# alshai/rowbowt

Measured on AMD Instinct MI355X. Metric: reads/s (100 bp, count+locate), higher is better.
Workload: dtype u32/u64

## Files before the change

rowbowt_amd/csrc/k_runs.hip:

```cpp
#include <type_traits>

#include "rbg_runs2_device.hpp"
#include "rbg_chain_walk.hpp"
#include "rbg_locate_docs.hpp"
#include "rbg_jump.h"
#include "rbg_launch.hpp"

namespace rbg {
namespace {

struct PackedBits {
    const uint4 *__restrict__ cp;
    uint4 w;
    uint32_t widx, navail;
    uint64_t sr;
    __device__ __forceinline__ uint32_t next_word() {
        if (widx == 4) { w = *cp++; widx = 0; }
        const uint32_t v = w.x;
        w.x = w.y; w.y = w.z; w.z = w.w;
        ++widx;
        return v;
    }
    __device__ __forceinline__ uint32_t take(uint32_t nb) {
        if (navail < nb) { sr |= static_cast<uint64_t>(next_word()) << navail; navail += 32; }
        const uint32_t v = static_cast<uint32_t>(sr & ((uint64_t(1) << nb) - 1));
        sr >>= nb;
        navail -= nb;
        return v;
    }
};

template <bool GLDS>
__device__ __forceinline__ bool jump_probe_wave(const void *__restrict__ tab, const uint64_t nb, const bool probing, const JumpKey &key, uint32_t v[3],
                                                uint32_t &buckets, lds_byte *tile) {
    uint32_t state = probing ? kJumpNext : kJumpAbsent;
    uint64_t b = probing ? jump_home(jump_hash(key), nb) : 0u;
    uint64_t left = nb;
    while (__ballot(state == kJumpNext)) {
        const bool undecided = state == kJumpNext;
        uint32_t w[16];
        quad_fetch_issue<GLDS>(reinterpret_cast<uint64_t>(tab) + (undecided ? b : 0u) * kJumpBucketBytes, w, tile);
        quad_fetch_take<GLDS>(w, tile);
        if (undecided) {
            ++buckets;
            state = jump_bucket(w, key, v);
            b = jump_next(b, nb);
            if (--left == 0 && state == kJumpNext) state = kJumpAbsent;
        }
    }
    return state <= kJumpHit1;
}

__device__ __forceinline__ uint64_t uniform_u64(const uint64_t v) {
    const uint32_t lo = static_cast<uint32_t>(__builtin_amdgcn_readfirstlane(static_cast<uint32_t>(v)));
    const uint32_t hi = static_cast<uint32_t>(__builtin_amdgcn_readfirstlane(static_cast<uint32_t>(v >> 32)));
    return static_cast<uint64_t>(lo) | (static_cast<uint64_t>(hi) << 32);
}

struct StagedWords {
    const lds_u32 *codes;
    __device__ __forceinline__ uint32_t operator()(const uint32_t j) const { return codes[64u * j]; }
};

template <typename P, bool TOEHOLD, bool PACKED = false, bool STATS = false, bool GLDS = false, bool STAGE = false>
__global__ __launch_bounds__(512, STATS ? 2 : 4) void k_find_range_runs(const DevIndex ix, const void *__restrict__ src_a,
                                                        const void *__restrict__ src_b, const uint64_t N,
                                                        uint64_t *__restrict__ lo_out, uint64_t *__restrict__ hi_out,
                                                        uint64_t *__restrict__ ss_out, unsigned long long *__restrict__ stats,
                                                        const uint32_t *__restrict__ sel, const uint32_t *__restrict__ nsel) {
    const uint64_t Neff = sel ? static_cast<uint64_t>(*nsel) : N;
    const uint8_t *__restrict__ seqs = static_cast<const uint8_t *>(src_a);
    const uint64_t *__restrict__ off = static_cast<const uint64_t *>(src_b);
    const uint4 *__restrict__ chunks = static_cast<const uint4 *>(src_a);
    const uint2 *__restrict__ meta = static_cast<const uint2 *>(src_b);
    __shared__ uint8_t s_lut[256];
    __shared__ uint8_t s_lut2[256];
    __shared__ uint8_t s_mslot[4];
    __shared__ __align__(16) unsigned char s_tile[GLDS ? 8 * kTileBytes : 16];
    __shared__ uint32_t s_codes[STAGE ? 8 * kStageWords * 64 : 1];
    __shared__ uint64_t s_jump[STAGE ? 4 : 1];
    __shared__ uint32_t s_jump_k[STAGE ? 2 : 1];
    for (int t = threadIdx.x; t < 256; t += blockDim.x) {
        s_lut[t] = ix.lut[t];
        s_lut2[t] = ix.nmajor ? ix.lut2[t] : 0xFFu;
    }
    if (STAGE && threadIdx.x < 2) {
        const uint32_t t = threadIdx.x;
        s_jump[2 * t] = reinterpret_cast<uint64_t>(ix.jump) + (t ? ix.jump_buckets * kJumpBucketBytes : 0u);
        s_jump[2 * t + 1] = t ? ix.jump2_buckets : ix.jump_buckets;
        s_jump_k[t] = t ? ix.jump2_k : ix.jump_k;
    }
    RBG_RUN_SEARCH2_SHARED;
    const RunSearch2<P> S2 = stage_run_search2<P>(ix, s_tab_first, s_ent2, s_dir2, s_rec2, s_dyn);
    const uint32_t *tab_first = s_tab_first;
    lds_byte *tile = (lds_byte *)s_tile + (GLDS ? (threadIdx.x >> 6) * kTileBytes : 0u);
    if (PACKED || STAGE) {
        for (int t = threadIdx.x; t < 256; t += blockDim.x)
            if (s_lut2[t] != 0xFFu) s_mslot[s_lut2[t] & 3u] = s_lut[t];
        __syncthreads();
    }
    const uint32_t D = ix.run_ksteps, DMASK = ix.run_depth_mask | 1u;
    const uint32_t M = ix.nmajor;
    const uint32_t lane = threadIdx.x & (kWave - 1);
    lds_u32 *codes = (lds_u32 *)s_codes + (STAGE ? (threadIdx.x >> 6) * (kStageWords * 64u) + lane : 0u);
    const StageTab stage_tab{ix.stage_code[0], ix.stage_code[1], ix.stage_byte[0], ix.stage_byte[1], ix.stage_shift};
    const bool stage_on = STAGE && ix.stage_ok != 0 && M == 4;

    unsigned long long c_occ = 0, c_reads = 0;
    uint32_t c_matched = 0;
    unsigned long long st[kStatSearchN] = {0, 0, 0, 0, 0, 0, 0, 0};
    const uint64_t stride = static_cast<uint64_t>(gridDim.x) * blockDim.x;
    const uint64_t wave_first = static_cast<uint64_t>(blockIdx.x) * blockDim.x + (threadIdx.x & ~(kWave - 1));
    for (uint64_t base = wave_first; base < Neff; base += stride) {
        bool valid = base + lane < Neff;
        const uint64_t i = (sel && valid) ? static_cast<uint64_t>(sel[base + lane]) : base + lane;
        uint64_t beg = 0, p = 0;
        PackedBits bs{chunks, make_uint4(0, 0, 0, 0), 4u, 0u, 0ull};
        if (PACKED) {
            if (valid) {
                const uint2 mt = meta[i];
                if (mt.y & 0x80000000u) valid = false;
                else { p = mt.y; bs.cp = chunks + mt.x; }
            }
        } else if (valid) { beg = off[i]; p = off[i + 1]; }
        bool staged = false;
        if constexpr (STAGE && !PACKED) {
            if (stage_on && __ballot(valid && p - beg > kStageCap) == 0) {
                uint32_t nch = 0;
                const bool bad = valid && stage_read(reinterpret_cast<const uint4 *>(seqs), beg, p, stage_tab, codes, nch);
                if (STATS) st[kStChunks] += nch;
                staged = __ballot(bad) == 0;
                if (staged) { p -= beg; beg = 0; }
                else if (STATS) st[kStChunks] -= nch;
            }
        }
        auto walk = [&](auto staged_tag) __attribute__((always_inline)) {
            constexpr bool STAGED = decltype(staged_tag)::value;
            const uint64_t p_end = p;
            uint64_t p_min = p;
            const uint32_t m32 = static_cast<uint32_t>(p);
            uint64_t lo = 0, hi = ix.n - 1;
            uint64_t k = TOEHOLD ? ix.last_run_sample : 0;
            bool alive = valid;
            bool pend = false;
            uint32_t pend_d = 0, pend_rec = 0;
            uint64_t pend_e = 0;
            ByteCursor rd{reinterpret_cast<const uint4 *>(seqs), ~uint64_t(0), make_uint4(0, 0, 0, 0)};
            bool jumped = false;
            if constexpr (STAGED && sizeof(P) == 4) {
                if (ix.jump) {
                    const uint32_t nlev = ix.jump2_k ? 2u : 1u;
                    bool hit = valid;
                    uint32_t from = 0;
#pragma unroll 1
                    for (uint32_t lev = 0; lev < nlev; ++lev) {
                        const uint32_t K = __builtin_amdgcn_readfirstlane(s_jump_k[lev]);
                        const uint64_t tab = uniform_u64(s_jump[2 * lev]), nb = uniform_u64(s_jump[2 * lev + 1]);
                        const bool probing = hit && static_cast<uint32_t>(p) >= K;
                        JumpKey key = jump_key_from_codes(StagedWords{codes}, from, K);
                        if (lev) key.w[3] = static_cast<uint32_t>(lo);
                        from = K;
                        uint32_t v[3] = {0, 0, 0}, nbk = 0;
                        hit = jump_probe_wave<GLDS>(reinterpret_cast<const void *>(tab), nb, probing, key, v, nbk, tile);
                        if (hit) {
                            lo = v[0]; hi = v[1];
                            if (TOEHOLD) k = v[2] == 0xFFFFFFFFu ? ~uint64_t(0) : static_cast<uint64_t>(v[2]);
                            p -= K;
                            jumped = true;
                            if (STATS) st[kStSymbols] += K;
                        }
                        if (STATS) st[kStFtab] += nbk;
                        if constexpr (!STATS) {
                            if (probing && !hit && jump_absent_ends(ix.jump_complete, lev)) { alive = false; p = beg; }
                        }
                    }
                }
            }
            if (!jumped && valid && ix.ftab_k && p - beg >= ix.ftab_k) {
                uint64_t idx = 0;
                bool all_major = true;
                PackedBits probe = bs;
                if constexpr (STAGED) {
                    const uint32_t w0 = codes[0];
                    idx = ix.ftab_k >= 16u ? w0 : (w0 & ((1u << (2u * ix.ftab_k)) - 1u));
                } else if (PACKED) {
                    idx = probe.take(2 * ix.ftab_k);
                } else {
                    uint64_t pw = 1;
                    for (uint32_t t = 1; t <= ix.ftab_k; ++t) {
                        const uint32_t mm = s_lut2[rd.at(p - t)];
                        all_major = all_major && mm != 0xFFu;
                        idx += (mm & 3u) * pw;
                        pw *= M;
                    }
                }
                uint64_t flo, fhi2, fk;
                if (STATS) { if (!STAGED) p_min = p - ix.ftab_k; if (all_major) st[kStFtab] += 1; }
                if (all_major && ftab_lookup<P>(ix, idx, flo, fhi2, fk)) {
// ... 79 lines not shown
                    if (STATS) st[kStSymbols] += adv;
                    const uint64_t c_inside = r.c_upto - r.c_before;
                    if (c_inside == 0) {
                        alive = false;
                    } else {
                        if (TOEHOLD) {
                            if (r.inside) k = k - adv;
                            else { pend = true; pend_d = d; pend_rec = rec; pend_e = r.samp_e; k = 0; }
                        }
                        lo = r.F + r.c_before;
                        hi = lo + c_inside - 1;
                        p = p_next;
                    }
                }
            }
            if (TOEHOLD && alive && pend) {
                k += run_step_sample2<P>(ix, S2, pend_d, pend_rec, pend_e);
                if (STATS) st[kStResample] += 1;
            }
            if (STATS && !PACKED && !STAGED && p_end > p_min) st[kStChunks] += ((p_end - 1) >> 4) - (p_min >> 4) + 1;
            if (STATS && PACKED && valid) st[kStChunks] += (p_end + 63) >> 6;
            if (!alive) { lo = 1; hi = 0; k = 0; }
            if (valid) {
                lo_out[i] = lo;
                hi_out[i] = hi;
                if (TOEHOLD) ss_out[i] = k;
                c_reads += 1;
                if (alive) { c_matched += 1; c_occ += hi - lo + 1; }
            }
        };
        if (STAGE && staged) walk(std::integral_constant<bool, STAGE>{}); else walk(std::false_type{});
    }
    c_reads = wave_sum(c_reads);
    const unsigned long long w_matched = wave_sum(static_cast<unsigned long long>(c_matched));
    c_occ = wave_sum(c_occ);
    if (lane == 0 && c_reads) {
        atomicAdd(&ix.counters[0], c_reads);
        if (w_matched) atomicAdd(&ix.counters[1], w_matched);
        if (c_occ) atomicAdd(&ix.counters[2], c_occ);
    }
    if (STATS) {
#pragma unroll
        for (int t = 0; t < kStatSearchN; ++t) {
            const unsigned long long v = wave_sum(st[t]);
            if (lane == 0 && v) atomicAdd(&stats[t], v);
        }
    }
}

template <typename P> struct ChunkR { static constexpr int v = 8; };

template <typename P, typename OUT = uint64_t, bool STATS = false, bool SUB = false, bool HI8 = false>
__global__ __launch_bounds__(256, 4) void k_locate_fill_runs2(const DevIndex ix, const uint64_t *__restrict__ lo,
                                                          const uint64_t *__restrict__ hi, const uint64_t *__restrict__ k,
                                                          const uint64_t N, const uint64_t max_hits,
                                                          const uint64_t *__restrict__ loc_off, OUT *__restrict__ locs,
                                                          const uint64_t *__restrict__ sub, const uint32_t *__restrict__ order,
                                                          const uint64_t *__restrict__ skeys, unsigned long long *__restrict__ stats) {
    constexpr int kChunkR = ChunkR<P>::v;
    using Stage = ChainStage<P, kChunkR, SUB, true, HI8>;
    __shared__ Stage S;
    chain_fill_walk<P, OUT, STATS, SUB, HI8, kChunkR, 1>(ix, S, lo, hi, k, N, max_hits, loc_off, locs, sub, order, skeys, stats,
                                                         [&](const uint64_t k1, unsigned long long &cost) { return run_phi<P, STATS>(ix, k1, cost); });
}

extern __shared__ unsigned long long locate_docs_lds[];
template <typename P, bool LOCS>
__global__ __launch_bounds__(kLocDocBlock) void k_locate_docs_runs2(const DevIndex ix, const DocTable t, const uint64_t *__restrict__ lo,
                                                                   const uint64_t *__restrict__ hi, const uint64_t *__restrict__ k, const uint64_t N,
                                                                   const uint64_t max_hits, const uint32_t *__restrict__ order,
                                                                   const uint64_t *__restrict__ skeys, uint64_t *__restrict__ sets,
                                                                   uint32_t *__restrict__ ndocs_out, uint32_t *__restrict__ nodoc_out,
                                                                   unsigned long long *__restrict__ doc_reads, unsigned long long *__restrict__ doc_locs) {
    locate_docs_walk<P, LOCS>(ix, t, locate_docs_lds, lo, hi, k, N, max_hits, order, skeys, sets, ndocs_out, nodoc_out, doc_reads, doc_locs,
                              [&](const uint64_t k1, unsigned long long &cost) { return run_phi<P>(ix, k1, cost); });
}

}

int launch_find_range_runs_impl(const DevIndex &ix, const LaunchCfg &cfg, const void *src_a, const void *src_b, uint64_t N,
                                uint64_t *lo, uint64_t *hi, uint64_t *ssamp, void *stream, bool packed, unsigned long long *stats,
                                const uint32_t *sel = nullptr, const uint32_t *nsel = nullptr) {
    if (N == 0) return 0;
    const size_t lds = run_search2_lds(ix);
    static const bool glds = [] { const char *e = std::getenv("RBG_REC_FETCH"); return !(e && std::strcmp(e, "quad") == 0); }();
    static const bool stage = [] { const char *e = std::getenv("RBG_STAGE_READS"); return !(e && e[0] == '0'); }();
    if (stats && packed) return static_cast<int>(hipErrorNotSupported);
    const LaunchCfg c = runs512_cfg(cfg);
    const dim3 grid(sel ? std::min(grid_for(c, N), 256) : grid_for(c, N)), block(512);
    return with_pos(ix.pos_bytes, [&](auto p) { return with_flag(ssamp != nullptr, [&](auto toe) {
        auto search = [&](auto pk, auto sts, auto gl, auto sg) {
            constexpr bool GL = decltype(gl)::value, SG = decltype(sg)::value;
            return launch_lds(k_find_range_runs<pos_t<decltype(p)>, decltype(toe)::value, decltype(pk)::value, decltype(sts)::value, GL, SG>, grid, block, lds,
                              (GL ? 8 * kTileBytes : 0) + (SG ? 8 * kStageWaveBytes : 0), stream, ix, src_a, src_b, N, lo, hi, ssamp, stats, sel, nsel);
        };
        auto fetch = [&](auto pk, auto sts) {
            if constexpr (!decltype(pk)::value) { if (glds && stage && !sel) return search(no, sts, yes, yes); }
            return glds ? search(pk, sts, yes, no) : search(pk, sts, no, no);
        };
        if (stats) return fetch(no, yes);
        return packed ? fetch(yes, no) : fetch(no, no);
    }); });
}

int launch_find_range_runs(const DevIndex &ix, const LaunchCfg &cfg, const uint8_t *seqs, const uint64_t *off, uint64_t N,
                           uint64_t *lo, uint64_t *hi, uint64_t *ssamp, void *stream, unsigned long long *stats) {
    return launch_find_range_runs_impl(ix, cfg, seqs, off, N, lo, hi, ssamp, stream, false, stats);
}

int launch_find_range_runs_sel(const DevIndex &ix, const LaunchCfg &cfg, const uint8_t *seqs, const uint64_t *off, uint64_t N, uint64_t *lo,
                               uint64_t *hi, uint64_t *ssamp, const uint32_t *sel, const uint32_t *nsel, void *stream) {
    return launch_find_range_runs_impl(ix, cfg, seqs, off, N, lo, hi, ssamp, stream, false, nullptr, sel, nsel);
}

int launch_find_range_runs_packed(const DevIndex &ix, const LaunchCfg &cfg, const uint2 *meta, const uint4 *chunks, uint64_t N,
                                  uint64_t *lo, uint64_t *hi, uint64_t *ssamp, void *stream) {
    return launch_find_range_runs_impl(ix, cfg, chunks, meta, N, lo, hi, ssamp, stream, true, nullptr);
}

int launch_locate_fill_runs(const DevIndex &ix, const LaunchCfg &cfg, const uint64_t *lo, const uint64_t *hi, const uint64_t *k,
                            uint64_t N, uint64_t max_hits, const uint64_t *loc_off, uint64_t *locs, const uint64_t *sub,
                            const void *order, const uint64_t *skeys, void *stream, unsigned long long *stats, uint32_t *locs32) {
    if (N == 0) return 0;
    const dim3 grid(grid_for(cfg, N)), block(256);
    const uint32_t *perm = static_cast<const uint32_t *>(order);
    return chain_fill_variants(ix, stats, sub, locs, locs32, [&](auto p, auto sts, auto sb, auto h8, auto *dst) {
        return launch_grid(k_locate_fill_runs2<pos_t<decltype(p)>, std::remove_pointer_t<decltype(dst)>, decltype(sts)::value, decltype(sb)::value, decltype(h8)::value>,
                           grid, block, 0, stream, ix, lo, hi, k, N, max_hits, loc_off, dst, sub, perm, skeys, stats);
    });
}

int launch_locate_doc_hits_runs(const DevIndex &ix, const DocTable &t, const uint64_t *lo, const uint64_t *hi, const uint64_t *k, uint64_t N, uint64_t max_hits,
                                const void *order, const uint64_t *skeys, uint64_t *sets, uint32_t *ndocs_out, uint32_t *nodoc_out, uint64_t *doc_reads,
                                uint64_t *doc_locs, void *stream) {
    if (t.ndocs == 0 || t.ndocs > kLocDocLdsDocs) return static_cast<int>(hipErrorInvalidValue);
    if (N == 0) return 0;
    const dim3 grid(locate_docs_grid(N)), block(kLocDocBlock);
    const uint32_t *perm = static_cast<const uint32_t *>(order);
    unsigned long long *dr = reinterpret_cast<unsigned long long *>(doc_reads), *dl = reinterpret_cast<unsigned long long *>(doc_locs);
    const size_t lds = locate_docs_lds_bytes(t.ndocs, t.ndir, doc_locs != nullptr);
    return with_pos(ix.pos_bytes, [&](auto p) { return with_flag(doc_locs != nullptr, [&](auto lc) {
        return launch_lds(k_locate_docs_runs2<pos_t<decltype(p)>, decltype(lc)::value>, grid, block, lds, 0, stream,
                          ix, t, lo, hi, k, N, max_hits, perm, skeys, sets, ndocs_out, nodoc_out, dr, dl);
    }); });
}

}
```

rowbowt_amd/csrc/rbg_dev.h:

```cpp
#pragma once

#include <hip/hip_runtime.h>

#include <algorithm>
#include <cstddef>
#include <cstdint>
#include <cstdio>
#include <vector>

#include "rbg_mkdir.hpp"
#include "rbg_fl.hpp"
#include "rbg_isa.hpp"

namespace rbg {

template <typename P>
struct RunEnt {
    P start;
    P cum;
};

template <typename P>
struct PhiEnt {
    P pos;
// ... 61 lines not shown
    uint32_t nruns;
};

constexpr int kLdsSyms = 8;
constexpr int kMaxMajor = 4;

struct DevRunTab2 {
    uint64_t F;
    uint64_t first;
    uint64_t dir_off;
    uint32_t dir_shift, pad;
};
static_assert(sizeof(DevRunTab2) == 32, "two 16-byte reads per record");
constexpr uint32_t kRunHotShiftBit = 56;
struct RunDir64 { uint32_t count, hi; };
constexpr uint32_t kRec2Pivots = 12;
constexpr uint32_t kRec2Overflow = 16u;
constexpr uint32_t kRec2Compact = 32u;
constexpr uint32_t kRec2CompactIn = 10;
struct alignas(64) RunRec2 {
    uint32_t e0;
    uint32_t hi;
    uint32_t meta;
    uint32_t cum_end;
    uint32_t ent[kRec2Pivots];
};
static_assert(sizeof(RunRec2) == 64, "one sector per bucket");
constexpr uint32_t kRunFillShift = 30;
struct PhiEnt12 { uint32_t pos_lo, base_lo, base_hi; };
static_assert(sizeof(PhiEnt12) == 12, "three words per entry");
constexpr uint32_t kPhiSuperShift = 16;

constexpr int kMaxRunDepth = 8;
constexpr int kLdsRunDepth = 5;
constexpr int kMaxLdsRunTabs = kLdsSyms + 16 + 64 + 256 + 1024 + kLdsRunDepth;


struct DevIndex {
    uint64_t n, r;
    uint64_t last_run_sample;
    const DevSym *syms;
    uint32_t sigma;
    uint32_t pos_bytes;
    const void *phi_ent;
    const void *phi_slots;
    const uint32_t *phi_ord;
    uint32_t phi_shift;
    uint32_t has_tsa;
    const uint64_t *mk_start, *mk_end, *mk_off, *mk_vals;
    uint64_t mk_nruns;
    const uint32_t *mk_bucket;
    uint32_t mk_shift;
    const MkRec *mk_rec;
    unsigned long long *counters;
    const uint8_t *lut;
    const DevSym *pairs;
    const DevSym *triples;
    const DevSym *quads;
    const DevSym *quints;
    const uint8_t *lut2;
    uint32_t nmajor;
    uint32_t kmer_steps;
    const void *ftab;
    uint32_t ftab_k;
    uint32_t phi_packed;
    const uint8_t *dense;
    uint32_t layout;
    uint32_t run_ksteps;
    uint32_t run_ntabs;
    const void *run_samp[kMaxRunDepth];
    uint32_t run_tab_first[kMaxRunDepth + 1];
    const uint32_t *phi_dir;
    uint32_t phi_dir_shift;
    uint32_t run_depth_mask;
    uint32_t phi_super_shift;
    uint32_t run_fill_shift;
    const void *run_ent2[kMaxRunDepth];
    const void *run_dir2[kMaxRunDepth];
    const DevRunTab2 *run_tabs2;
    const uint64_t *run_hot;
    uint32_t run_uni_depth;
    uint32_t run_uni_stride;
    uint32_t run_uni_shift;
    const RunRec2 *run_rec2[kMaxRunDepth];
    const uint64_t *phi_super;
    uint64_t phi_m;
    uint64_t phi_last_pos, phi_last_base;
    const uint64_t *order_docs;
    uint32_t order_ndocs, order_dbits, order_lowbits, order_obits;
    uint32_t stage_ok, stage_shift;
    uint32_t stage_code[2];
    uint32_t stage_byte[2];
    const void *jump;
    uint64_t jump_buckets;
    uint32_t jump_k;
    uint32_t jump2_k;
    uint64_t jump2_buckets;
    uint32_t jump_complete;
    uint32_t tmk_shift;
    const uint64_t *tmk_start, *tmk_end, *tmk_off, *tmk_vals;
    uint64_t tmk_nruns;
    const uint32_t *tmk_bucket;
    const MkRec *tmk_rec;
};

enum SearchStat {
    kStSteps = 0,
    kStSlots,
    kStDense,
    kStSearch,
    kStFtab,
    kStResample,
    kStChunks,
    kStSymbols,
    kStatSearchN
};
static_assert(kMkStatRuns == kStatSearchN + 2, "marker_span_arrays counts the run starts / ends it reads behind the search counters");
enum LocateStat {
    kLsPhiSteps = 0,
    kLsPhiOvf,
    kLsChains,
    kLsLocs,
    kStatLocateN
};

template <typename P>
struct SeedLogRec {
    P lo, hi;
    uint32_t qs, qe, mb, me;
};
struct SeedLogWin {
    uint32_t src, cnt;
};
struct SeedLog {
    unsigned char *base;
    uint64_t stride;
    uint32_t qs, qw;
    uint32_t *nsel;
    unsigned long long *stats = nullptr;
};
enum SeedStat {
    kSdMarkerQueries = kStatSearchN,
    kSdMarkerDir,
    kSdMarkerProbes,
    kSdMarkerOff,
    kSdMarkerVals,
    kSdSeedRecs,
    kSdSequences,
    kSeedStatN
};
constexpr uint32_t kSeedLogOverflow = 0xFFFFFFFFu;
constexpr uint32_t kSeedLogWindows = 6, kSeedLogSeedsDefault = 12;
inline size_t seed_log_rec_bytes(uint32_t pos_bytes) { return pos_bytes == 4 ? sizeof(SeedLogRec<uint32_t>) : sizeof(SeedLogRec<uint64_t>); }
inline size_t seed_log_stride(uint32_t pos_bytes, uint32_t seeds_per_read) {
    return 8 + static_cast<size_t>(seeds_per_read) * seed_log_rec_bytes(pos_bytes) + kSeedLogWindows * sizeof(SeedLogWin);
}
inline size_t seed_log_bytes(uint64_t N, uint32_t pos_bytes, uint32_t seeds_per_read) {
    return static_cast<size_t>(N) * seed_log_stride(pos_bytes, seeds_per_read) + 64 + (N + 4) * 4;
}
inline SeedLog make_seed_log(void *scratch, size_t bytes, uint64_t N, uint32_t pos_bytes) {
    SeedLog lg{nullptr, 0, 0, kSeedLogWindows, nullptr, nullptr};
    if (!scratch || N == 0 || (reinterpret_cast<uintptr_t>(scratch) & 15)) return lg;
    const size_t tail = 64 + (N + 4) * 4, fixed = 8 + kSeedLogWindows * sizeof(SeedLogWin), rec = seed_log_rec_bytes(pos_bytes);
    if (bytes < tail + N * (fixed + 2 * rec)) return lg;
    size_t q = ((bytes - tail) / N - fixed) / rec;
    if (q > 255) q = 255;
    lg.qs = static_cast<uint32_t>(q);
    lg.stride = fixed + q * rec;
    lg.base = static_cast<unsigned char *>(scratch);
    lg.nsel = reinterpret_cast<uint32_t *>(lg.base + ((N * lg.stride + 15) & ~size_t(15)));
    return lg;
}

struct ComposeTable {
    const void *ent;
    const void *samp;
    uint64_t nruns, total, F;
};
struct ComposedLevel {
    void *ent = nullptr;
    void *samp = nullptr;
    uint64_t entries = 0;
    std::vector<uint64_t> nruns, total, F, first;
};
int compose_levels_device(uint32_t pos_bytes, uint64_t n, uint32_t M, const ComposeTable *major, const void *g_start, const uint32_t *g_id,
                          const void *g_samp, uint64_t g_n, uint32_t kmax, bool with_samples, std::vector<ComposedLevel> &out, void *stream,
                          uint32_t keep_mask = 0 ,
                          bool *inputs_released = nullptr );

inline double host_memory_available() {
    double avail = 1e18;
    if (FILE *f = std::fopen("/proc/meminfo", "r")) {
        char line[256];
        while (std::fgets(line, sizeof line, f)) {
            unsigned long long kb = 0;
            if (std::sscanf(line, "MemAvailable: %llu kB", &kb) == 1) { avail = static_cast<double>(kb) * 1024.0; break; }
        }
        std::fclose(f);
    }
    unsigned long long mx = 0, cur = 0;
    bool have_mx = false, have_cur = false;
    if (FILE *f = std::fopen("/sys/fs/cgroup/memory.max", "r")) { have_mx = std::fscanf(f, "%llu", &mx) == 1; std::fclose(f); }
    if (FILE *f = std::fopen("/sys/fs/cgroup/memory.current", "r")) { have_cur = std::fscanf(f, "%llu", &cur) == 1; std::fclose(f); }
    if (have_mx && have_cur && mx > cur) avail = std::min(avail, static_cast<double>(mx - cur));
    else if (have_mx && have_cur) avail = 0;
    return avail;
}


struct LaunchCfg {
    int block_threads = 256;
    int max_blocks = 0;
};

int launch_find_range(const DevIndex &ix, const LaunchCfg &cfg, const uint8_t *seqs, const uint64_t *off, uint64_t N,
                      uint64_t *lo, uint64_t *hi, uint64_t *ssamp , void *stream);
int launch_find_range_runs(const DevIndex &ix, const LaunchCfg &cfg, const uint8_t *seqs, const uint64_t *off, uint64_t N,
                           uint64_t *lo, uint64_t *hi, uint64_t *ssamp , void *stream,
                           unsigned long long *stats = nullptr );
int launch_find_range_runs_sel(const DevIndex &ix, const LaunchCfg &cfg, const uint8_t *seqs, const uint64_t *off, uint64_t N, uint64_t *lo,
                               uint64_t *hi, uint64_t *ssamp , const uint32_t *sel, const uint32_t *nsel, void *stream);
int launch_find_range_runs_packed(const DevIndex &ix, const LaunchCfg &cfg, const uint2 *meta, const uint4 *chunks, uint64_t N,
                                  uint64_t *lo, uint64_t *hi, uint64_t *ssamp , void *stream);
int launch_locate_fill_runs(const DevIndex &ix, const LaunchCfg &cfg, const uint64_t *lo, const uint64_t *hi, const uint64_t *k,
                            uint64_t N, uint64_t max_hits, const uint64_t *loc_off, uint64_t *locs, const uint64_t *sub,
                            const void *order, const uint64_t *skeys, void *stream, unsigned long long *stats = nullptr ,
                            uint32_t *locs32 = nullptr);
int launch_lf_runs(const DevIndex &ix, const LaunchCfg &cfg, const uint64_t *lo, const uint64_t *hi, const uint8_t *sym, uint64_t N,
                   uint64_t *lo_out, uint64_t *hi_out, void *stream);
int launch_find_range_markers_runs(const DevIndex &ix, const LaunchCfg &cfg, const uint8_t *seqs, const uint64_t *off, uint64_t N,
                                   uint64_t wsize, uint64_t max_range, uint64_t *lo, uint64_t *hi, uint64_t *cnt, const uint64_t *mk_off,
                                   uint64_t *mk, bool fill, void *stream);
int launch_greedy_seed_runs(const DevIndex &ix, const LaunchCfg &cfg, const uint8_t *seqs, const uint64_t *off, uint64_t N,
                            uint64_t min_length, uint64_t *lo, uint64_t *hi, uint64_t *qs, uint64_t *qe, uint64_t *ss, void *stream,
                            unsigned long long *stats = nullptr );
int launch_marker_seeds_runs(const DevIndex &ix, const LaunchCfg &cfg, const uint8_t *seqs, const uint64_t *off, uint64_t N, uint64_t wsize,
                             uint64_t max_range, uint64_t *seed_cnt, uint64_t *mk_cnt, const uint64_t *seed_off, const uint64_t *mk_off,
                             uint64_t *seeds, uint64_t *mk, bool fill, void *stream, const SeedLog &lg, uint64_t ftab_k = 0 );
int launch_marker_lmems_runs(const DevIndex &ix, const LaunchCfg &cfg, const uint8_t *seqs, const uint64_t *off, uint64_t N, uint64_t total,
                             uint64_t wsize, uint64_t max_range, uint64_t ftab_k, uint64_t *rec_off, uint64_t *seeds, uint64_t *mk, bool fill,
                             void *stream);
int launch_greedy_seeds_list_runs(const DevIndex &ix, const LaunchCfg &cfg, const uint8_t *seqs, const uint64_t *off, uint64_t N, uint64_t min_length,
                                  bool w_sample, uint64_t *seed_cnt, const uint64_t *seed_off, uint64_t *lo, uint64_t *hi, uint64_t *qs, uint64_t *qe,
                                  uint64_t *ss , bool fill, void *stream);
int launch_toehold_chkpnts_runs(const DevIndex &ix, const LaunchCfg &cfg, const uint8_t *seqs, const uint64_t *off, uint64_t N, uint64_t wsize,
                                const uint64_t *slot_off, uint64_t *cnt, uint64_t *lo, uint64_t *hi, uint64_t *qs, uint64_t *qe, uint64_t *ss,
                                void *stream);
int launch_find_range_stats(const DevIndex &ix, const LaunchCfg &cfg, const uint8_t *seqs, const uint64_t *off, uint64_t N,
                            uint64_t *lo, uint64_t *hi, uint64_t *ssamp , unsigned long long *stats ,
                            void *stream);
size_t scan_tmp_bytes(uint64_t N);
int launch_locate_plan(const DevIndex &ix, const LaunchCfg &cfg, const uint64_t *lo, const uint64_t *hi, uint64_t N,
                       uint64_t max_hits, uint64_t *loc_off, void *tmp, size_t tmp_bytes, void *stream);
int launch_locate_fill(const DevIndex &ix, const LaunchCfg &cfg, const uint64_t *lo, const uint64_t *hi,
                       const uint64_t *k, uint64_t N, uint64_t max_hits, const uint64_t *loc_off, uint64_t *locs,
                       const uint64_t *sub ,
                       const void *order , void *stream,
                       unsigned long long *stats = nullptr ,
                       uint32_t *locs32 = nullptr );
size_t locate_order_ws_bytes(uint64_t N);
int launch_locate_order(const DevIndex &ix, const LaunchCfg &cfg, const uint64_t *k, uint64_t N, void *ws, size_t ws_bytes,
                        void *stream);
int launch_build_rank_slots(uint32_t pos_bytes, const void *ent, uint64_t nruns, uint64_t n, uint32_t shift, void *slots,
                            uint32_t *ord, unsigned long long *overflow, unsigned long long *dense_cursor, void *stream);
int launch_fill_dense(uint32_t pos_bytes, const void *ent, uint64_t n, uint32_t shift, const void *slots, const uint32_t *ord,
                      uint8_t *dense, void *stream);
size_t text_ws_bytes(uint64_t E);
int launch_copy16(const void *pinned_src, void *dst, uint64_t bytes, void *stream);
int launch_text_plan(const uint64_t *lo, const uint64_t *hi, const uint64_t *loc_off, const uint64_t *locs, uint64_t N, uint64_t E, const char *names,
                     const uint32_t *name_off, const uint64_t *doc_start, const char *doc_names, const uint32_t *doc_name_off, uint64_t ndocs,
                     uint64_t text_size, bool with_locs, const uint64_t *mk_off, const uint64_t *mk, void *ws, size_t ws_bytes, unsigned int *d_bad, void *stream);
void text_total_ptrs(void *ws, uint64_t E, const uint64_t **last_at, const uint32_t **last_len);
int launch_text_fill(const uint64_t *lo, const uint64_t *hi, const uint64_t *loc_off, const uint64_t *locs, uint64_t N, uint64_t E, const char *names,
                     const uint32_t *name_off, const uint64_t *doc_start, const char *doc_names, const uint32_t *doc_name_off, uint64_t ndocs,
                     uint64_t text_size, bool with_locs, const uint64_t *mk_off, const uint64_t *mk, void *ws, uint64_t total, char *text, void *stream);
struct SamBatch {
    uint64_t N, E;
    const uint64_t *lo, *hi, *a, *b;
    const uint8_t *rev;
    const uint64_t *line_off, *loc_off, *locs;
    const char *seqs, *quals;
    const uint64_t *roff;
    const char *names;
    const uint32_t *name_off;
    const uint64_t *doc_start;
    const char *doc_names;
    const uint32_t *doc_name_off;
    uint64_t ndocs, text_size;
};
int launch_sam_strands(const uint8_t *seqs, const uint64_t *off, uint64_t N, uint64_t total, uint8_t *out, uint64_t *off2, uint32_t cap, void *stream);
size_t sam_pick_tmp_bytes(uint64_t N);
int launch_sam_pick(const uint64_t *lo2, const uint64_t *hi2, const uint64_t *qs2, const uint64_t *qe2, const uint64_t *ss2, uint64_t N, uint64_t max_hits,
                    uint64_t *lo, uint64_t *hi, uint64_t *k, uint64_t *a, uint64_t *b, uint8_t *rev, uint64_t *nlines, uint64_t *line_off,
                    unsigned long long *counters, void *tmp, size_t tmp_bytes, uint32_t cap, void *stream);
size_t sam_ws_bytes(uint64_t E);
int launch_sam_plan(const SamBatch &B, void *ws, size_t ws_bytes, unsigned int *d_bad, uint32_t cap, void *stream);
void sam_total_ptrs(void *ws, uint64_t E, const uint64_t **last_at, const uint64_t **last_len);
int launch_sam_fill(const SamBatch &B, void *ws, uint64_t total, char *text, uint32_t cap, void *stream);
int launch_sam_offsets(void *ws, uint64_t E, void *stream);
int launch_extend_left(const DevIndex &ix, const uint8_t *seqs, const uint64_t *off, uint64_t N, const uint32_t *item_seq, const uint32_t *item_a,
                       const uint64_t *item_row, const uint64_t *item_limit, uint64_t M, uint32_t max_mismatch, void *out, unsigned int *d_err, uint32_t cap,
                       void *stream);
// ... 160 lines not shown
```

rowbowt_amd/csrc/rbg_jump.h:

```cpp
#pragma once

#include <cstdint>

#if defined(__HIPCC__)
#define RBG_JUMP_HD __host__ __device__ __forceinline__
#else
#define RBG_JUMP_HD inline
#endif

namespace rbg {

constexpr uint32_t kJumpMaxK = 64;
constexpr uint32_t kJumpMinK = 16;
constexpr uint32_t kJumpSlotWords = 8;
constexpr uint32_t kJumpBucketBytes = 64;
constexpr uint32_t kJumpEmptyTag = 0, kJumpFullTag = 1;
constexpr uint32_t kJumpDefaultK = 60;
constexpr uint64_t kJumpAutoMinBytes = uint64_t(256) << 20;

struct JumpKey {
    uint32_t w[4];
};

RBG_JUMP_HD void jump_key_mask(JumpKey &key, uint32_t K) {
// ... 9 lines not shown
}

RBG_JUMP_HD uint64_t jump_hash(const JumpKey &key) {
    const uint64_t a = key.w[0] | (static_cast<uint64_t>(key.w[1]) << 32);
    const uint64_t b = key.w[2] | (static_cast<uint64_t>(key.w[3]) << 32);
    uint64_t h = (a * 0x9E3779B97F4A7C15ull) ^ ((b + 0x632BE59BD9B4E019ull) * 0xC2B2AE3D27D4EB4Full);
    h ^= h >> 29;
    h *= 0xBF58476D1CE4E5B9ull;
    h ^= h >> 32;
    return h;
}

RBG_JUMP_HD uint64_t jump_home(uint64_t h, uint64_t nb) {
    return ((h >> 32) * nb) >> 32;
}

constexpr uint32_t kJumpHit0 = 0, kJumpHit1 = 1, kJumpAbsent = 2, kJumpNext = 3;
RBG_JUMP_HD uint32_t jump_bucket(const uint32_t w[16], const JumpKey &key, uint32_t v[3]) {
    for (uint32_t s = 0; s < 2; ++s) {
        const uint32_t *sl = w + kJumpSlotWords * s;
        if (sl[7] == kJumpEmptyTag) return kJumpAbsent;
        if (sl[0] == key.w[0] && sl[1] == key.w[1] && sl[2] == key.w[2] && sl[3] == key.w[3]) {
            v[0] = sl[4]; v[1] = sl[5]; v[2] = sl[6];
            return s;
        }
    }
    return kJumpNext;
}

RBG_JUMP_HD uint64_t jump_next(uint64_t b, uint64_t nb) { return b + 1 == nb ? 0 : b + 1; }

template <typename Load>
RBG_JUMP_HD bool jump_probe(const Load &load, uint64_t nb, const JumpKey &key, uint32_t v[3], uint32_t &buckets) {
    uint64_t b = jump_home(jump_hash(key), nb);
    for (uint64_t step = 0; step < nb; ++step) {
        ++buckets;
        uint32_t w[16];
        load(b, 0, w, w + 4);
        load(b, 1, w + 8, w + 12);
        const uint32_t r = jump_bucket(w, key, v);
        if (r != kJumpNext) return r != kJumpAbsent;
        b = jump_next(b, nb);
    }
    return false;
}

constexpr uint32_t kJump2MaxK = 48;
constexpr uint32_t kJump2MinK = 16;
constexpr uint32_t kJump2DefaultK = 40;

RBG_JUMP_HD JumpKey jump2_key(uint32_t s0, uint32_t s1, uint32_t s2, uint32_t K2, uint32_t parent_lo) {
    JumpKey key{{s0, s1, s2, 0u}};
    jump_key_mask(key, K2);
    key.w[3] = parent_lo;
    return key;
}

template <typename Word>
RBG_JUMP_HD JumpKey jump_key_from_codes(const Word &word, uint32_t from, uint32_t K) {
    const uint32_t w0 = from >> 4, sh = 2u * (from & 15u);
    const uint32_t c0 = word(w0), c1 = word(w0 + 1), c2 = word(w0 + 2), c3 = word(w0 + 3), c4 = word(w0 + 4);
    const auto funnel = [sh](uint32_t lo, uint32_t hi) { return static_cast<uint32_t>(((static_cast<uint64_t>(hi) << 32) | lo) >> sh); };
    JumpKey key{{funnel(c0, c1), funnel(c1, c2), funnel(c2, c3), funnel(c3, c4)}};
    jump_key_mask(key, K);
    return key;
}

template <typename Word>
RBG_JUMP_HD JumpKey jump2_key_from_codes(const Word &word, uint32_t K1, uint32_t K2, uint32_t parent_lo) {
    JumpKey key = jump_key_from_codes(word, K1, K2);
    key.w[3] = parent_lo;
    return key;
}

RBG_JUMP_HD JumpKey jump2_key_from_text(const uint8_t *codes, uint32_t K2, uint32_t parent_lo) {
    JumpKey key{{0, 0, 0, 0}};
    for (uint32_t t = 0; t < K2; ++t) jump_key_set(key, t, codes[K2 - 1 - t]);
    key.w[3] = parent_lo;
    return key;
}

inline uint64_t jump_buckets_for(uint64_t keys) { return keys ? keys : 1; }

constexpr uint32_t kJumpComplete1 = 1u, kJumpComplete2 = 2u;
struct JumpBuilt {
    bool stands;
    uint64_t words, inserted;
};
RBG_JUMP_HD bool jump_level_complete(const JumpBuilt &b) { return b.stands && b.words != 0 && b.inserted == b.words; }
RBG_JUMP_HD uint32_t jump_complete_mask(const JumpBuilt &l1, const JumpBuilt &l2, bool absent_ends) {
    if (!absent_ends || !l1.stands) return 0u;
    return (jump_level_complete(l1) ? kJumpComplete1 : 0u) | (jump_level_complete(l2) ? kJumpComplete2 : 0u);
}
RBG_JUMP_HD bool jump_absent_ends(uint32_t mask, uint32_t lev) { return ((mask >> lev) & 1u) != 0; }

}
```

Before: 2.417 billion.

## Add lean two-level jump-table kernel for exact-length reads, defer rest to runs search

Adds a small, high-occupancy kernel that handles reads whose length equals K1+K2. It stages each read into LDS, probes the two complete jump hash tables, and writes the range directly. Reads it cannot take are marked with a sentinel. The full runs search kernel then runs in a marked-only mode that skips already-resolved reads, using a reduced persistent grid. This trades one extra launch and an extra pass over lo_out for avoiding the heavy backward-search kernel on most 100 bp reads.

New measurement: 2.370 billion. -1.9%, worse.

```diff
diff --git a/rowbowt_amd/csrc/jump_lean.hip b/rowbowt_amd/csrc/jump_lean.hip
--- /dev/null
+++ b/rowbowt_amd/csrc/jump_lean.hip
@@ -0,0 +1,97 @@
+#include "rbg_jump_probe.hpp"
+#include "rbg_launch.hpp"
+
+namespace rbg {
+namespace {
+
+constexpr int kLeanBlock = 256;
+constexpr uint32_t kLeanWords = 8u;
+static_assert((kJumpMaxK + kJump2MaxK + 15u) / 16u <= kLeanWords, "a read the lean kernel takes fits its column");
+
+struct LeanColumn {
+    const lds_u32 *codes;
+    __device__ __forceinline__ uint32_t operator()(const uint32_t j) const { return codes[64u * j]; }
+};
+
+struct LeanIndex {
+    const void *tab1, *tab2;
+    uint64_t nb1, nb2;
+    uint32_t K1, K2;
+    StageTab stage;
+    unsigned long long *counters;
+};
+
+template <bool TOEHOLD>
+__global__ __launch_bounds__(kLeanBlock, 8) void k_jump_lean(const LeanIndex ix, const uint8_t *__restrict__ seqs, const uint64_t *__restrict__ off,
+                                                             const uint64_t N, uint64_t *__restrict__ lo_out, uint64_t *__restrict__ hi_out,
+                                                             uint64_t *__restrict__ ss_out) {
+    __shared__ uint32_t s_codes[(kLeanBlock / kWave) * kLeanWords * 64];
+    const uint32_t lane = threadIdx.x & (kWave - 1);
+    lds_u32 *codes = (lds_u32 *)s_codes + (threadIdx.x >> 6) * (kLeanWords * 64u) + lane;
+    const uint32_t K1 = ix.K1, K2 = ix.K2;
+    unsigned long long c_occ = 0;
+    uint32_t c_reads = 0, c_matched = 0;
+    const uint64_t stride = static_cast<uint64_t>(gridDim.x) * blockDim.x;
+    const uint64_t wave_first = static_cast<uint64_t>(blockIdx.x) * blockDim.x + (threadIdx.x & ~(kWave - 1));
+    for (uint64_t base = wave_first; base < N; base += stride) {
+        const uint64_t i = base + lane;
+        const bool valid = i < N;
+        uint64_t beg = 0, end = 0;
+        if (valid) { beg = off[i]; end = off[i + 1]; }
+        bool take = valid && jump_lean_takes(end - beg, K1, K2);
+        uint64_t lo = 1, hi = 0, k = 0;
+        bool hit = false;
+        if (__ballot(take)) {
+            uint32_t nch = 0;
+            const bool bad = stage_read(reinterpret_cast<const uint4 *>(seqs), take ? beg : 0u, take ? end : 0u, ix.stage, codes, nch);
+            take = take && !bad;
+            const JumpWordsClamped<LeanColumn> words{LeanColumn{codes}, kLeanWords};
+            uint32_t v[3] = {0, 0, 0}, nbk = 0;
+            const JumpKey key1 = jump_key_from_codes(words, 0u, K1);
+            hit = jump_probe_wave<false>(ix.tab1, ix.nb1, take, key1, v, nbk, nullptr);
+            const JumpKey key2 = jump2_key_from_codes(words, K1, K2, v[0]);
+            hit = jump_probe_wave<false>(ix.tab2, ix.nb2, hit, key2, v, nbk, nullptr);
+            if (hit) {
+                lo = v[0]; hi = v[1];
+                if (TOEHOLD) k = v[2] == 0xFFFFFFFFu ? ~uint64_t(0) : static_cast<uint64_t>(v[2]);
+            }
+        }
+        if (valid) {
+            if (!take) {
+                lo_out[i] = kJumpDeferMark;
+            } else {
+                lo_out[i] = lo;
+                hi_out[i] = hi;
+                if (TOEHOLD) ss_out[i] = k;
+                c_reads += 1;
+                if (hit) { c_matched += 1; c_occ += hi - lo + 1; }
+            }
+        }
+    }
+    const unsigned long long w_reads = wave_sum(static_cast<unsigned long long>(c_reads));
+    const unsigned long long w_matched = wave_sum(static_cast<unsigned long long>(c_matched));
+    c_occ = wave_sum(c_occ);
+    if (lane == 0 && w_reads) {
+        atomicAdd(&ix.counters[0], w_reads);
+        if (w_matched) atomicAdd(&ix.counters[1], w_matched);
+        if (c_occ) atomicAdd(&ix.counters[2], c_occ);
+    }
+}
+
+}
+
+int launch_jump_lean(const DevIndex &ix, const LaunchCfg &cfg, const uint8_t *seqs, const uint64_t *off, uint64_t N, uint64_t *lo, uint64_t *hi,
+                     uint64_t *ssamp, void *stream) {
+    if (N == 0) return 0;
+    if (!jump_lean_index_ok(ix.jump != nullptr, ix.jump2_k, ix.jump_complete, ix.stage_ok, ix.nmajor, ix.pos_bytes)) return static_cast<int>(hipErrorInvalidValue);
+    LaunchCfg c = cfg;
+    c.block_threads = kLeanBlock;
+    const dim3 grid(grid_for(c, N)), block(kLeanBlock);
+    const LeanIndex L{ix.jump, static_cast<const char *>(ix.jump) + ix.jump_buckets * kJumpBucketBytes, ix.jump_buckets, ix.jump2_buckets, ix.jump_k, ix.jump2_k,
+                      StageTab{ix.stage_code[0], ix.stage_code[1], ix.stage_byte[0], ix.stage_byte[1], ix.stage_shift}, ix.counters};
+    return with_flag(ssamp != nullptr, [&](auto toe) {
+        return launch_grid(k_jump_lean<decltype(toe)::value>, grid, block, 0, stream, L, seqs, off, N, lo, hi, ssamp);
+    });
+}
+
+}
diff --git a/rowbowt_amd/csrc/k_runs.hip b/rowbowt_amd/csrc/k_runs.hip
--- a/rowbowt_amd/csrc/k_runs.hip
+++ b/rowbowt_amd/csrc/k_runs.hip
@@ -4,6 +4,7 @@
 #include "rbg_chain_walk.hpp"
 #include "rbg_locate_docs.hpp"
 #include "rbg_jump.h"
+#include "rbg_jump_probe.hpp"
 #include "rbg_launch.hpp"
 
 namespace rbg {
@@ -30,26 +31,6 @@
     }
 };
 
-template <bool GLDS>
-__device__ __forceinline__ bool jump_probe_wave(const void *__restrict__ tab, const uint64_t nb, const bool probing, const JumpKey &key, uint32_t v[3],
-                                                uint32_t &buckets, lds_byte *tile) {
-    uint32_t state = probing ? kJumpNext : kJumpAbsent;
-    uint64_t b = probing ? jump_home(jump_hash(key), nb) : 0u;
-    uint64_t left = nb;
-    while (__ballot(state == kJumpNext)) {
-        const bool undecided = state == kJumpNext;
-        uint32_t w[16];
-        quad_fetch_issue<GLDS>(reinterpret_cast<uint64_t>(tab) + (undecided ? b : 0u) * kJumpBucketBytes, w, tile);
-        quad_fetch_take<GLDS>(w, tile);
-        if (undecided) {
-            ++buckets;
-            state = jump_bucket(w, key, v);
-            b = jump_next(b, nb);
-            if (--left == 0 && state == kJumpNext) state = kJumpAbsent;
-        }
-    }
-    return state <= kJumpHit1;
-}
 
 __device__ __forceinline__ uint64_t uniform_u64(const uint64_t v) {
     const uint32_t lo = static_cast<uint32_t>(__builtin_amdgcn_readfirstlane(static_cast<uint32_t>(v)));
@@ -114,6 +95,12 @@
     for (uint64_t base = wave_first; base < Neff; base += stride) {
         bool valid = base + lane < Neff;
         const uint64_t i = (sel && valid) ? static_cast<uint64_t>(sel[base + lane]) : base + lane;
+        if constexpr (sizeof(P) == 4 && !PACKED && !STATS) {
+            if (ix.marked_only) {
+                if (valid) valid = lo_out[i] == kJumpDeferMark;
+                if (__ballot(valid) == 0) continue;
+            }
+        }
         uint64_t beg = 0, p = 0;
         PackedBits bs{chunks, make_uint4(0, 0, 0, 0), 4u, 0u, 0ull};
         if (PACKED) {
@@ -359,12 +346,14 @@
                                 uint64_t *lo, uint64_t *hi, uint64_t *ssamp, void *stream, bool packed, unsigned long long *stats,
                                 const uint32_t *sel = nullptr, const uint32_t *nsel = nullptr) {
     if (N == 0) return 0;
+    const bool marked = ix.marked_only != 0;
     const size_t lds = run_search2_lds(ix);
     static const bool glds = [] { const char *e = std::getenv("RBG_REC_FETCH"); return !(e && std::strcmp(e, "quad") == 0); }();
     static const bool stage = [] { const char *e = std::getenv("RBG_STAGE_READS"); return !(e && e[0] == '0'); }();
     if (stats && packed) return static_cast<int>(hipErrorNotSupported);
     const LaunchCfg c = runs512_cfg(cfg);
-    const dim3 grid(sel ? std::min(grid_for(c, N), 256) : grid_for(c, N)), block(512);
+    const int looping = sel ? 256 : std::max(1, c.max_blocks / 8);
+    const dim3 grid(sel || marked ? std::min(grid_for(c, N), looping) : grid_for(c, N)), block(512);
     return with_pos(ix.pos_bytes, [&](auto p) { return with_flag(ssamp != nullptr, [&](auto toe) {
         auto search = [&](auto pk, auto sts, auto gl, auto sg) {
             constexpr bool GL = decltype(gl)::value, SG = decltype(sg)::value;
@@ -382,6 +371,15 @@
 
 int launch_find_range_runs(const DevIndex &ix, const LaunchCfg &cfg, const uint8_t *seqs, const uint64_t *off, uint64_t N,
                            uint64_t *lo, uint64_t *hi, uint64_t *ssamp, void *stream, unsigned long long *stats) {
+    static const bool lean = [] { const char *e = std::getenv("RBG_JUMP_LEAN"); return !(e && e[0] == '0'); }();
+    static const bool stage = [] { const char *e = std::getenv("RBG_STAGE_READS"); return !(e && e[0] == '0'); }();
+    if (lean && stage && !stats && N != 0 &&
+        jump_lean_index_ok(ix.jump != nullptr, ix.jump2_k, ix.jump_complete, ix.stage_ok, ix.nmajor, ix.pos_bytes)) {
+        if (const int rc = launch_jump_lean(ix, cfg, seqs, off, N, lo, hi, ssamp, stream)) return rc;
+        DevIndex rest = ix;
+        rest.marked_only = 1u;
+        return launch_find_range_runs_impl(rest, cfg, seqs, off, N, lo, hi, ssamp, stream, false, nullptr);
+    }
     return launch_find_range_runs_impl(ix, cfg, seqs, off, N, lo, hi, ssamp, stream, false, stats);
 }
 
diff --git a/rowbowt_amd/csrc/rbg_dev.h b/rowbowt_amd/csrc/rbg_dev.h
--- a/rowbowt_amd/csrc/rbg_dev.h
+++ b/rowbowt_amd/csrc/rbg_dev.h
@@ -167,6 +167,7 @@
     uint32_t run_uni_depth;
     uint32_t run_uni_stride;
     uint32_t run_uni_shift;
+    uint32_t marked_only;
     const RunRec2 *run_rec2[kMaxRunDepth];
     const uint64_t *phi_super;
     uint64_t phi_m;
@@ -303,6 +304,8 @@
 int launch_find_range_runs(const DevIndex &ix, const LaunchCfg &cfg, const uint8_t *seqs, const uint64_t *off, uint64_t N,
                            uint64_t *lo, uint64_t *hi, uint64_t *ssamp , void *stream,
                            unsigned long long *stats = nullptr );
+int launch_jump_lean(const DevIndex &ix, const LaunchCfg &cfg, const uint8_t *seqs, const uint64_t *off, uint64_t N, uint64_t *lo, uint64_t *hi,
+                     uint64_t *ssamp , void *stream);
 int launch_find_range_runs_sel(const DevIndex &ix, const LaunchCfg &cfg, const uint8_t *seqs, const uint64_t *off, uint64_t N, uint64_t *lo,
                                uint64_t *hi, uint64_t *ssamp , const uint32_t *sel, const uint32_t *nsel, void *stream);
 int launch_find_range_runs_packed(const DevIndex &ix, const LaunchCfg &cfg, const uint2 *meta, const uint4 *chunks, uint64_t N,
diff --git a/rowbowt_amd/csrc/rbg_jump.h b/rowbowt_amd/csrc/rbg_jump.h
--- a/rowbowt_amd/csrc/rbg_jump.h
+++ b/rowbowt_amd/csrc/rbg_jump.h
@@ -115,6 +115,13 @@
 
 inline uint64_t jump_buckets_for(uint64_t keys) { return keys ? keys : 1; }
 
+template <typename Word>
+struct JumpWordsClamped {
+    Word word;
+    uint32_t nwords;
+    RBG_JUMP_HD uint32_t operator()(uint32_t j) const { return j < nwords ? word(j) : 0u; }
+};
+
 constexpr uint32_t kJumpComplete1 = 1u, kJumpComplete2 = 2u;
 struct JumpBuilt {
     bool stands;
@@ -127,4 +134,10 @@
 }
 RBG_JUMP_HD bool jump_absent_ends(uint32_t mask, uint32_t lev) { return ((mask >> lev) & 1u) != 0; }
 
+constexpr uint64_t kJumpDeferMark = ~uint64_t(0);
+RBG_JUMP_HD bool jump_lean_takes(uint64_t m, uint32_t K1, uint32_t K2) { return m == static_cast<uint64_t>(K1) + K2; }
+RBG_JUMP_HD bool jump_lean_index_ok(bool has1, uint32_t k2, uint32_t complete, uint32_t stage_ok, uint32_t nmajor, uint32_t pos_bytes) {
+    return has1 && k2 != 0 && complete == (kJumpComplete1 | kJumpComplete2) && stage_ok != 0 && nmajor == 4 && pos_bytes == 4;
 }
+
+}
diff --git a/rowbowt_amd/csrc/rbg_jump_probe.hpp b/rowbowt_amd/csrc/rbg_jump_probe.hpp
--- /dev/null
+++ b/rowbowt_amd/csrc/rbg_jump_probe.hpp
@@ -0,0 +1,31 @@
+#pragma once
+
+#include "rbg_runs2_device.hpp"
+#include "rbg_jump.h"
+
+namespace rbg {
+namespace {
+
+template <bool GLDS>
+__device__ __forceinline__ bool jump_probe_wave(const void *__restrict__ tab, const uint64_t nb, const bool probing, const JumpKey &key, uint32_t v[3],
+                                                uint32_t &buckets, lds_byte *tile) {
+    uint32_t state = probing ? kJumpNext : kJumpAbsent;
+    uint64_t b = probing ? jump_home(jump_hash(key), nb) : 0u;
+    uint64_t left = nb;
+    while (__ballot(state == kJumpNext)) {
+        const bool undecided = state == kJumpNext;
+        uint32_t w[16];
+        quad_fetch_issue<GLDS>(reinterpret_cast<uint64_t>(tab) + (undecided ? b : 0u) * kJumpBucketBytes, w, tile);
+        quad_fetch_take<GLDS>(w, tile);
+        if (undecided) {
+            ++buckets;
+            state = jump_bucket(w, key, v);
+            b = jump_next(b, nb);
+            if (--left == 0 && state == kJumpNext) state = kJumpAbsent;
+        }
+    }
+    return state <= kJumpHit1;
+}
+
+}
+}
```
